# shunkenney/DPE-MVS

Hardware: AMD Instinct MI355X
Metric: depth-map Mpixels/sec (9-view 1600x1200 PatchMatch) at 1/2/4/8 GPUs; L1 vs ref (higher is better)
Workload: dtype f32; 1 GPU; DTU-like 1600x1200, 9 src views, full-res REFINE_ITER pass + geometric consistency (BASELINE configs[2]); width=1600, height=1200, num_images=10, parallelism=reference-image sharding x1

## Files before the change

dpe-mvs_amd/csrc/lds_layout.h:

```cpp
#pragma once

#if defined(__HIPCC__)
#define LDS_HD __host__ __device__
#else
#define LDS_HD
#endif

namespace dpe {
namespace lds {

constexpr int kMaxViews = 31;

struct Region {
  int off, len, align;
};

template <int N>
constexpr bool regions_ok(const Region (&r)[N], int total) {
  for (int i = 0; i < N; ++i) {
    if (r[i].len < 0 || r[i].off < 0 || r[i].off + r[i].len > total) return false;
    if (r[i].align > 1 && r[i].off % r[i].align != 0) return false;
    for (int j = i + 1; j < N; ++j)
      if (r[i].len > 0 && r[j].len > 0 && r[i].off < r[j].off + r[j].len && r[j].off < r[i].off + r[i].len) return false;
  }
// ... 4 lines not shown
struct StrongCarve {
  static constexpr int kPatch = 108;
  LDS_HD static constexpr int ib_ints(int nv) { return 2 * C + 17 + nv; }
  LDS_HD static constexpr int hyp() { return 0; }
  LDS_HD static constexpr int patch() { return P * 20; }
  LDS_HD static constexpr int cost(int) { return P * 128; }
  LDS_HD static constexpr int sp(int nv) { return P * (128 + (C + 1) * nv); }
  LDS_HD static constexpr int ref(int nv) { return P * (128 + (C + 2) * nv); }
  LDS_HD static constexpr int fc(int nv) { return P * (128 + (C + 7) * nv); }
  LDS_HD static constexpr int sums(int nv) { return P * (136 + (C + 7) * nv); }
  LDS_HD static constexpr int vw(int nv) { return P * (140 + (C + 7) * nv); }
  LDS_HD static constexpr int ib(int nv) { return P * (148 + (C + 7) * nv); }
  LDS_HD static constexpr int base(int nv) { return (ib(nv) + P * ib_ints(nv) + 3) & ~3; }
  LDS_HD static constexpr int cpl(int nv) { return base(nv); }
  LDS_HD static constexpr int alias(int nv) { return base(nv) + P * (C + 1) * 4; }
  LDS_HD static constexpr int tail(int nv) { return alias(nv) + P * (C + 1); }
  LDS_HD static constexpr int rnd(int nv) { return tail(nv) + TAIL_JOBS * 18; }
  LDS_HD static constexpr int total(int nv) { return rnd(nv) + P * 12; }
  static constexpr int IB_POS = 0;
  static constexpr int IB_FIN = C;
  static constexpr int IB_MISC = C + 8;
  static constexpr int IB_SEL = C + 16;
  LDS_HD static constexpr int ib_slots(int nv) { return C + 16 + nv; }
  static constexpr int MI_NSEL = 0, MI_JOBS = 1, MI_DEPTH = 2;

  static constexpr bool ok(int nv) {
    const Region r[] = {{hyp(), P * 20, 4},        {patch(), P * kPatch, 1}, {cost(nv), P * (C + 1) * nv, 1},
                        {sp(nv), P * nv, 1},       {ref(nv), P * 5 * nv, 1}, {fc(nv), P * 8, 1},
                        {sums(nv), P * 4, 1},      {vw(nv), P * 8, 1},       {ib(nv), P * ib_ints(nv), 1},
                        {cpl(nv), P * (C + 1) * 4, 4}, {alias(nv), P * (C + 1), 1}, {tail(nv), TAIL_JOBS * 18, 1},
                        {rnd(nv), P * 12, 1}};
    return regions_ok(r, total(nv)) && ib_slots(nv) + C + 1 == ib_ints(nv) && P * C == 64 && MI_DEPTH + 5 <= 8;
  }
  static constexpr bool ok_all() {
    for (int nv = 1; nv <= kMaxViews; ++nv) if (!ok(nv)) return false;
    return true;
  }
};

template <bool PRE>
struct WeakCarveT {
  static constexpr int PW = 0;
  static constexpr int TC = 108;
  static constexpr int TN = 180;
  static constexpr int SUMS = 324;
  static constexpr int RC = 351;
  static constexpr int OSUM = 352;
  static constexpr int CPL = 356;
  static constexpr int HYP = 388;
  static constexpr int RSUM = HYP;
  static constexpr int FC = 416;
  static constexpr int MISC = 424;
  static constexpr int NBL = 440;
  static constexpr int NBOX_A = 449;
  static constexpr int NSV = 452;
  static constexpr int NBOX_B = 461;
  static constexpr int ALIAS = PRE ? 472 : 464;
  static constexpr int VWL = PRE ? 464 : 472;
  static constexpr int RND = 472;
  static constexpr int FIXED = PRE ? 484 : 480;
  static constexpr int M_NSEL = 0, M_RADC = 1, M_INCC = 2, M_NC = 3, M_WNORM = 4, M_CMASK = 5, M_NB3 = 6, M_POOL = 7, M_FLAGS = 8;
  LDS_HD static constexpr int cost(int) { return FIXED; }
  LDS_HD static constexpr int sp(int nv) { return FIXED + 8 * nv; }
  LDS_HD static constexpr int sel(int nv) { return FIXED + 9 * nv; }
  LDS_HD static constexpr int hv(int nv) { return FIXED + 10 * nv; }
  LDS_HD static constexpr int per_pixel(int nv) { return (FIXED + 17 * nv + 3) & ~3; }

  static constexpr bool ok(int nv) {
    const Region r[] = {{PW, 108, 1},   {TC, 72, 1},      {TN, 144, 1},    {SUMS, 27, 1},       {RC, 1, 1},
                        {OSUM, 3, 1},   {CPL, 32, 4},     {HYP, 28, 4},    {FC, 8, 1},          {MISC, 16, 1},
                        {NBL, 9, 1},    {NBOX_A, 3, 1},   {NSV, 9, 1},     {NBOX_B, 1, 1},
                        {PRE ? RND : ALIAS, PRE ? 12 : 8, 1},
                        {VWL, 8, 1},    {cost(nv), 8 * nv, 1}, {sp(nv), nv, 1}, {sel(nv), nv, 1}, {hv(nv), 7 * nv, 1}};
    return regions_ok(r, per_pixel(nv)) && per_pixel(nv) % 4 == 0 && M_FLAGS + 8 <= 16 &&
           (!PRE || (ALIAS >= RND && ALIAS + 8 <= RND + 12));
  }
  static constexpr bool ok_all() {
    for (int nv = 1; nv <= kMaxViews; ++nv) if (!ok(nv)) return false;
    return true;
  }
};
using WeakCarve = WeakCarveT<false>;

static_assert(StrongCarve<4, 16, 16>::ok_all(), "strong-sweep LDS carve (edge mode): overlap, alignment or bounds");
static_assert(StrongCarve<8, 8, 16>::ok_all(), "strong-sweep LDS carve (ACMH mode): overlap, alignment or bounds");
static_assert(WeakCarveT<false>::ok_all(), "weak-sweep LDS carve: overlap, alignment or bounds");
static_assert(WeakCarveT<true>::ok_all(), "weak-sweep LDS carve (DPE_WEAK_PRE): overlap, alignment or bounds");
static_assert(4 * StrongCarve<4, 16, 16>::total(kMaxViews) * 4 <= 160 * 1024, "strong-sweep workgroup LDS (edge)");
static_assert(4 * StrongCarve<8, 8, 16>::total(kMaxViews) * 4 <= 160 * 1024, "strong-sweep workgroup LDS (ACMH)");
static_assert(4 * (4 * 4 * WeakCarveT<false>::per_pixel(9) * 4) <= 160 * 1024, "weak-sweep LDS: 4 workgroups per CU at 9 views");
static_assert(4 * (4 * 4 * WeakCarveT<true>::per_pixel(9) * 4) <= 160 * 1024, "weak-sweep LDS (DPE_WEAK_PRE): 4 workgroups per CU at 9 views");

}
}
```

dpe-mvs_amd/csrc/pass_common.h:

```cpp
#pragma once
#include "device_math.h"
#include "bres_walk.h"
#include "../../include/dpe_mvs.h"

namespace dpe {

struct ViewConst { float M[9]; float b[3]; };

struct PassConst {
  int W, H, N, LW, LH;
  int half_rows;
  uint32_t seed32, salt;
  float kinv0, kinv4, kc2, kc5;
  float gn_cos, gn_sin, gn_thr;
  int gn_shift;
  uint32_t gn_shift_m;
  int weak_nn;
  DpePatchMatchParams P;
  DpeCamera cams[DPE_MAX_IMAGES];
  ViewConst vc[DPE_MAX_IMAGES];
};

struct DevBufs {
  const float4* imgq[DPE_MAX_IMAGES];
  const uint8_t* img8; uint32_t img8_view;
// ... 200 lines not shown
}
DEV float4 random_normal_from(const DpeCamera& c, int px, int py, const float* n0, float depth) {
  float4 n = make_float4(n0[0], n0[1], n0[2], 0.0f);
  const float4 vd = view_direction(c, px, py, depth);
  if (n.x * vd.x + n.y * vd.y + n.z * vd.z > 0.0f) { n.x = -n.x; n.y = -n.y; n.z = -n.z; }
  normalize3(n);
  return n;
}
DEV float4 perturbed_normal_from(const DpeCamera& c, int px, int py, const float4& normal, const float* sc) {
  const float4 vd = view_direction(c, px, py, 1.0f);
  const float s1 = sc[0], c1 = sc[1], s2 = sc[2], c2 = sc[3], s3 = sc[4], c3 = sc[5];
  const float R0 = c2 * c3, R1 = c3 * s1 * s2 - c1 * s3, R2 = s1 * s3 + c1 * c3 * s2;
  const float R3 = c2 * s3, R4 = c1 * c3 + s1 * s2 * s3, R5 = c1 * s2 * s3 - c3 * s1;
  const float R6 = -s2, R7 = c2 * s1, R8 = c1 * c2;
  float4 np = make_float4(R0 * normal.x + R1 * normal.y + R2 * normal.z,
                          R3 * normal.x + R4 * normal.y + R5 * normal.z,
                          R6 * normal.x + R7 * normal.y + R8 * normal.z, normal.w);
  if (np.x * vd.x + np.y * vd.y + np.z * vd.z >= 0.0f) np = normal;
  normalize3(np);
  return np;
}

struct Homog { float h[9]; };
DEV Homog make_homography(const PassConst& pc, int v, const float4& pl) {
  const float iw = 1.0f / pl.w;
  const float qx = pl.x * iw, qy = pl.y * iw, qz = pl.z * iw;
  const float g0 = qx * pc.kinv0;
  const float g1 = qy * pc.kinv4;
  const float g2 = __builtin_fmaf(-qx, pc.kc2, __builtin_fmaf(-qy, pc.kc5, qz));
  const ViewConst& vc = pc.vc[v];
  Homog H;
  H.h[0] = __builtin_fmaf(-vc.b[0], g0, vc.M[0]);
  H.h[1] = __builtin_fmaf(-vc.b[0], g1, vc.M[1]);
  H.h[2] = __builtin_fmaf(-vc.b[0], g2, vc.M[2]);
  H.h[3] = __builtin_fmaf(-vc.b[1], g0, vc.M[3]);
  H.h[4] = __builtin_fmaf(-vc.b[1], g1, vc.M[4]);
  H.h[5] = __builtin_fmaf(-vc.b[1], g2, vc.M[5]);
  H.h[6] = __builtin_fmaf(-vc.b[2], g0, vc.M[6]);
  H.h[7] = __builtin_fmaf(-vc.b[2], g1, vc.M[7]);
  H.h[8] = __builtin_fmaf(-vc.b[2], g2, vc.M[8]);
  return H;
}
DEV float2 project_h(const Homog& H, float x, float y) {
  const float px = __builtin_fmaf(H.h[1], y, __builtin_fmaf(H.h[0], x, H.h[2]));
  const float py = __builtin_fmaf(H.h[4], y, __builtin_fmaf(H.h[3], x, H.h[5]));
  const float pz = __builtin_fmaf(H.h[7], y, __builtin_fmaf(H.h[6], x, H.h[8]));
  const float iz = 1.0f / pz;
  return make_float2(px * iz, py * iz);
}

DEV bool rcp_range_ok(const Homog& H, float x0, float x1, float y0, float y1) {
  const float b0 = __builtin_fmaf(H.h[6], x0, H.h[8]), b1 = __builtin_fmaf(H.h[6], x1, H.h[8]);
  const float q00 = __builtin_fmaf(H.h[7], y0, b0), q01 = __builtin_fmaf(H.h[7], y1, b0);
  const float q10 = __builtin_fmaf(H.h[7], y0, b1), q11 = __builtin_fmaf(H.h[7], y1, b1);
  const float mn = __builtin_fminf(__builtin_fminf(q00, q01), __builtin_fminf(q10, q11));
  const float mx = __builtin_fmaxf(__builtin_fmaxf(q00, q01), __builtin_fmaxf(q10, q11));
  const float amax = __builtin_fmaxf(__builtin_fmaxf(__builtin_fabsf(b0), __builtin_fabsf(b1)),
                                     __builtin_fmaxf(__builtin_fabsf(mn), __builtin_fabsf(mx)));
  const float lo = mn > 0.0f ? mn : -mx;
  return (mn > 0.0f || mx < 0.0f) && lo > amax * 9.5367431640625e-07f && lo > 7.888609052210118e-31f &&
         amax < 1.2676506002282294e+30f;
}

DEV bool taps_unclamped(const Homog& H, float x0, float x1, float y0, float y1, float wm1, float hm1) {
  const float b0 = __builtin_fmaf(H.h[6], x0, H.h[8]), b1 = __builtin_fmaf(H.h[6], x1, H.h[8]);
// ... 298 lines not shown
  if (rcp_range_ok(H, (float)(cx - radius), (float)(cx + radius), (float)(cy - radius), (float)(cy + radius)))
    generic_taps<U8, true>(pc, B, v, H, cx, cy, rcp, radius, increment, a);
  else
    generic_taps<U8, false>(pc, B, v, H, cx, cy, rcp, radius, increment, a);
  if (B.cnt) { const unsigned long long n = (unsigned long long)(2 * radius / increment + 1); count_work(B, 0, n * n); }
  return ncc_finalize(a[0], a[1], a[5], a[2], a[3], a[4]);
}

DEV float2 project_h_fast(const Homog& H, float x, float y) {
  const float px = __builtin_fmaf(H.h[1], y, __builtin_fmaf(H.h[0], x, H.h[2]));
  const float py = __builtin_fmaf(H.h[4], y, __builtin_fmaf(H.h[3], x, H.h[5]));
  const float pz = __builtin_fmaf(H.h[7], y, __builtin_fmaf(H.h[6], x, H.h[8]));
  const float iz = d_rcp_fast(pz);
  return make_float2(px * iz, py * iz);
}
template <bool FAST = false>
DEV bool center_outside(const PassConst& pc, int v, const Homog& H, int px, int py) {
  const float2 pt = FAST ? project_h_fast(H, (float)px, (float)py) : project_h(H, (float)px, (float)py);
  const DpeCamera& sc = pc.cams[v];
  return pt.x >= (float)sc.width || pt.x < 0.0f || pt.y >= (float)sc.height || pt.y < 0.0f;
}

template <int U8>
DEV float ncc_old_generic(const PassConst& pc, const DevBufs& B, int px, int py, int v, const float4& pl) {
  const Homog H = make_homography(pc, v, pl);
  count_work(B, 1, 0);
  if (center_outside(pc, v, H, px, py)) return 2.0f;
  const float rc = ref_texel(B.ref, pc.W, pc.H, px, py);
  return patch_ncc_generic<U8>(pc, B, v, H, px, py, rc, pc.P.strong_radius, pc.P.strong_increment);
}

struct Patch36 {
  float w[36], wr[36];
  float s_ref, s_rr, s_w;
  int px, py;
};
DEV void make_patch36(Patch36& P, const PassConst& pc, const DevBufs& B, int px, int py) {
  const int W = pc.W, Hh = pc.H;
  const float ss = pc.P.sigma_spatial, sc = pc.P.sigma_color;
  const float rc = ref_texel(B.ref, W, Hh, px, py);
  P.px = px; P.py = py;
  float s_ref = 0, s_rr = 0, s_w = 0;
#pragma unroll
  for (int a = 0; a < 6; ++a) {
    const int i = -5 + 2 * a;
    float r_ref = 0, r_rr = 0, r_w = 0;
#pragma unroll
    for (int b = 0; b < 6; ++b) {
      const int j = -5 + 2 * b;
      const float rp = ref_texel(B.ref, W, Hh, px + i, py + j);
      const float w = bilateral_weight(i, j, rp, rc, ss, sc);
      const float wr = w * rp;
// ... 173 lines not shown
```

dpe-mvs_amd/csrc/pass_refine.h:

```cpp
#pragma once
#include "pass_common.h"

namespace dpe {

DEV void wave_sync() {
  __builtin_amdgcn_fence(__ATOMIC_RELEASE, "wavefront");
  __builtin_amdgcn_wave_barrier();
  __builtin_amdgcn_fence(__ATOMIC_ACQUIRE, "wavefront");
}

template <int S>
DEV void patch_lds_build(float* pw, const PassConst& pc, const DevBufs& B, int px, int py, int t) {
  constexpr int R = (36 + S - 1) / S;
  const float rc = ref_texel(B.ref, pc.W, pc.H, px, py);
  float rp[R];
#pragma unroll
  for (int r = 0; r < R; ++r) {
    const int k = t + r * S < 36 ? t + r * S : 35;
    rp[r] = ref_texel(B.ref, pc.W, pc.H, px - 5 + 2 * (k / 6), py - 5 + 2 * (k % 6));
  }
#pragma unroll
  for (int r = 0; r < R; ++r) {
    const int k = t + r * S;
    if (k >= 36) break;
// ... 117 lines not shown
    r3[0] = r_sr.x; r3[1] = r_ss; r3[2] = r_sr.y;
  } else {
    const float bx = __builtin_fmaf(H.h[0], x, H.h[2]) * kTexUnit;
    const float by = __builtin_fmaf(H.h[3], x, H.h[5]) * kTexUnit;
    const float bz = __builtin_fmaf(H.h[6], x, H.h[8]);
    float r_src = 0, r_ss = 0, r_rs = 0;
#pragma unroll
    for (int b = 0; b < 6; ++b) {
      const float y = (float)(py - 5 + 2 * b);
      const float qx = __builtin_fmaf(H.h[1], y, bx);
      const float qy = __builtin_fmaf(H.h[4], y, by);
      const float iz = rcp_tap<FAST>(__builtin_fmaf(H.h[7], y, bz));
      const float sp = sample_src<U8>(B, v, W, Hh, qx, qy, iz);
      const float w = pw[2 * (a * 6 + b)], wr = pw[2 * (a * 6 + b) + 1];
      r_src = __builtin_fmaf(w, sp, r_src);
      const float ws = w * sp;
      r_ss = __builtin_fmaf(ws, sp, r_ss);
      r_rs = __builtin_fmaf(wr, sp, r_rs);
    }
    r3[0] = r_src; r3[1] = r_ss; r3[2] = r_rs;
  }
}
template <int U8>
DEV float ncc_old_lds(const float* pw, float s_ref, float s_rr, float s_w, int px, int py, const PassConst& pc,
                      const DevBufs& B, int v, const float4& pl) {
  const Homog H = make_homography(pc, v, pl);
  if (center_outside(pc, v, H, px, py)) { count_work(B, 1, 0); return 2.0f; }
  count_work(B, 1, 36);
  float a[3];
  const bool ok = rcp_range_ok(H, (float)(px - 5), (float)(px + 5), (float)(py - 5), (float)(py + 5));
  PATCH_STAT(ok);
  if (ok) {
    const bool ncl = taps_unclamped(H, (float)(px - 5), (float)(px + 5), (float)(py - 5), (float)(py + 5), (float)(pc.W - 1),
                                    (float)(pc.H - 1));
#if DPE_POOL_STATS
    atomicAdd(&g_pool[6][2], ncl ? 0ull : 1ull);
    atomicAdd(&g_pool[7][0], 1ull);
#endif
    if (DPE_UNCLAMPED && U8 != TEX_F32 && __all(ncl)) {
#if DPE_POOL_STATS
      atomicAdd(&g_pool[7][1], 1ull);
#endif
      lds_taps<U8, true, false>(pw, px, py, pc, B, v, H, a);
    } else
      lds_taps<U8, true>(pw, px, py, pc, B, v, H, a);
  } else
    lds_taps<U8, false>(pw, px, py, pc, B, v, H, a);
  return ncc_finalize_pre(s_ref, s_rr, s_w, a[0], a[1], a[2]);
}

template <int U8>
DEV float ncc_old_any(bool fast, const float* pw, float s_ref, float s_rr, float s_w, int px, int py,
                      const PassConst& pc, const DevBufs& B, int v, const float4& pl) {
  if (fast) return ncc_old_lds<U8>(pw, s_ref, s_rr, s_w, px, py, pc, B, v, pl);
  return ncc_old_generic<U8>(pc, B, px, py, v, pl);
}

DEV void baseline_and_weights(const PassConst& pc, uint32_t sel, const uint8_t* vw, float& base_line, float& weight_normal,
                              int& valid) {
  const DpeCamera& c0 = pc.cams[0];
  base_line = 0.0f; weight_normal = 0.0f; valid = 0;
  for (int si = 1; si < pc.N; ++si) {
    const int vi = si - 1;
    if (isSet(sel, vi)) {
      weight_normal += vw[vi];
      const DpeCamera& cs = pc.cams[si];
      const float d0 = c0.c[0] - cs.c[0], d1 = c0.c[1] - cs.c[1], d2 = c0.c[2] - cs.c[2];
      const float tv = d0 * d0 + d1 * d1 + d2 * d2;
      base_line += __builtin_sqrtf(tv);
      valid++;
    }
  }
}

DEV uint8_t d2w_class(const PassConst& pc, const float* pcs, uint64_t is_peak) {
  const int radius = 30;
  const int peak_count = __popcll(is_peak);
  int min_peak = 0;
// ... 319 lines not shown
```

dpe-mvs_amd/csrc/pass_sweep.h:

```cpp
#pragma once
#include "pass_common.h"
#include "pass_refine.h"
#include "lds_layout.h"

namespace dpe {

template <int MODE> constexpr int list_count() { return MODE == 0 ? 4 : 1; }
template <int MODE> DEV int list_rows(const PassConst& pc) { return MODE == 1 ? pc.H : pc.half_rows; }
template <int MODE> DEV int list_key(const PassConst& pc, const DevBufs& B, int x, int y) {
  if constexpr (MODE == 2) return (((x + y) & 1) == 0 && B.weak_rel[y * pc.W + x] == 0) ? 0 : -1;
  const bool wk = B.weak[y * pc.W + x] == DPE_WEAK;
  if constexpr (MODE == 1) return wk ? 0 : -1;
  else return (((x + y) & 1) << 1) | (wk ? 1 : 0);
}
template <int MODE>
__global__ void k_list_count(const PassConst* __restrict__ pcp, DevBufs B, int* __restrict__ row_counts) {
  constexpr int NL = list_count<MODE>();
  const PassConst& pc = *pcp;
  const int wave = threadIdx.x >> 6, lane = threadIdx.x & 63;
  const int y = blockIdx.x * 4 + wave, rows = list_rows<MODE>(pc);
  if (y >= rows) return;
  int cnt[NL];
  for (int j = 0; j < NL; ++j) cnt[j] = 0;
  for (int x0 = 0; x0 < pc.W; x0 += 64) {
// ... 298 lines not shown
      return cmp;
    }
  }
}

constexpr int kTailJobs = 16;
template <int P, int C> using StrongCarveT = lds::StrongCarve<P, C, kTailJobs>;
__host__ __device__ inline int strong_lds_per_wave(int P, int C, int nv) {
  return P == 4 && C == 16 ? StrongCarveT<4, 16>::total(nv) : StrongCarveT<8, 8>::total(nv);
}

template <int P>
DEV bool job_decode(const int* cnt, int j, int& p, int& r) {
  r = j;
#pragma unroll
  for (int q = 0; q < P; ++q) {
    if (r < cnt[q]) { p = q; return true; }
    r -= cnt[q];
  }
  return false;
}

constexpr int kBwStrong = 2;
template <int U8, bool EDGE>
__global__ void __launch_bounds__(64 * kBwStrong, kTapWaves) k_strong_coop(const PassConst* __restrict__ pcp, DevBufs B, int iter,
                                                     const int* __restrict__ list, const int* __restrict__ nlist_p) {
  extern __shared__ float4 lds4[];
  float* lds = (float*)lds4;
  const int nlist = *nlist_p;
  constexpr int C = EDGE ? 16 : 8;
  constexpr int P = 64 / C;
  const PassConst& pc = *pcp;
  const int wave = threadIdx.x >> 6, lane = threadIdx.x & 63;
  const int ps = lane / C, c = lane % C;
  const int W = pc.W, nv = pc.N - 1;
  const DpeCamera& c0 = pc.cams[0];
  const int wbase = (xcd_remap(blockIdx.x, gridDim.x, B.xcd_rows * 16) * kBwStrong + wave) * P;
  if (wbase >= nlist) return;
  const int gi = wbase + ps;
  const bool active = gi < nlist;
  const int center = active ? list[gi] : 0;
  const int x = center % W, y = center / W;
  using SC = StrongCarveT<P, C>;
  float* wl = lds + (size_t)wave * SC::total(nv);
  float4* hyp_all = (float4*)(wl + SC::hyp());
  float* pw_all = wl + SC::patch();
// ... 27 lines not shown
  bool on_edge = false;
  PHASE_BEGIN();
  if (active) {
    if (fast) patch_lds_build<C>(pw, pc, B, x, y, c);
    PHASE(14);
    int pos;
    if constexpr (EDGE) {
      on_edge = B.edge[center] != 0;
      const int d = c & 7, kind = c >> 3;
      pos = (kind == 1 && on_edge) ? -1 : edge_candidate(pc, B, costs_s, x, y, center, iter, d, kind, on_edge);
    } else {
      pos = acmh_candidate(pc, costs_s, x, y, center, c);
    }
    posl[c] = pos;
    auto phash = [](const float4& p) -> int {
      uint32_t h = __float_as_uint(p.x) * 0x9E3779B1u;
      h = (h ^ (h >> 15) ^ __float_as_uint(p.y)) * 0x85EBCA77u;
      h = (h ^ (h >> 13) ^ __float_as_uint(p.z)) * 0xC2B2AE3Du;
      h = (h ^ (h >> 16) ^ __float_as_uint(p.w)) * 0x27D4EB2Fu;
      return (int)((h ^ (h >> 15)) & 0x7FFFFFFFu);
    };
    if (pos >= 0) { const float4 pl = planes_s[pos]; cpl[c] = pl; alias[c] = phash(pl); }
    else alias[c] = (int)(0x80000000u | (uint32_t)c);
    if (c == 0) { const float4 pl = planes_s[center]; cpl[C] = pl; alias[C] = phash(pl); }
  }
  wave_sync();
  PHASE(0);
  auto same = [](const float4& a, const float4& b) {
    return __float_as_uint(a.x) == __float_as_uint(b.x) && __float_as_uint(a.y) == __float_as_uint(b.y) &&
           __float_as_uint(a.z) == __float_as_uint(b.z) && __float_as_uint(a.w) == __float_as_uint(b.w);
  };
  int al[2] = {-1, -1};
  if (active) {
#pragma unroll
    for (int r = 0; r < 2; ++r) {
      const int sl = c + r * C;
      if (sl > C || (sl < C && posl[sl] < 0)) continue;
      const float4 me = cpl[sl];
      const uint32_t h = (uint32_t)alias[sl];
      uint32_t m = 0;
#pragma unroll
      for (int t = 0; t < C; ++t) m |= ((uint32_t)alias[t] == h && t < sl) ? (1u << t) : 0u;
      int a = sl;
      while (m) {
        const int t = __builtin_ctz(m);
        if (same(cpl[t], me)) { a = t; break; }
        m &= m - 1;
      }
      al[r] = a;
    }
  }
  wave_sync();
  if (active) {
    alias[c] = al[0];
    if (c == 0) alias[C] = al[1];
  }
  wave_sync();
  PHASE(1);
  if (c == 0) {
    int n = 0;
    if (active) {
      for (int k = 0; k <= C; ++k) if (alias[k] == k) slots[n++] = k;
      if (fast) patch_lds_pre(pw, sums_all[ps * 4 + 0], sums_all[ps * 4 + 1], sums_all[ps * 4 + 2]);
    }
    misc[SC::MI_JOBS] = n;
  }
  wave_sync();
  PHASE(2);
  {
    int cnt[P], S = 0;
#pragma unroll
    for (int q = 0; q < P; ++q) { cnt[q] = ib_all[q * ibs + SC::IB_MISC + 1]; S += cnt[q]; }
    int q, r;
    const int total = S * nv, tail = total & 63;
    const bool split = fast && tail > 0 && tail <= kTailJobs;
    POOL_STAT(0, total);
    const int jend = split ? total - tail : total;
    for (int j = lane; j < jend; j += 64) {
      job_decode<P>(cnt, j % S, q, r);
      const int* iq = ib_all + q * ibs;
      const int slot = iq[SC::ib_slots(nv) + r], v = j / S + 1;
      const int cq = list[wbase + q];
      const int qx = cq % W, qy = cq / W;
      const float4 pl = cpl_all[q * (C + 1) + slot];
      const float* sm = sums_all + q * 4;
      cost_all[(q * (C + 1) + slot) * nv + v - 1] =
          ncc_old_any<U8>(fast, pw_all + q * 108, sm[0], sm[1], sm[2], qx, qy, pc, B, v, pl);
    }
    if (split) {
      float* tb = wl + SC::tail(nv);
      const int rpp = 64 / tail >= 6 ? 1 : 2, npc = 6 / rpp;
      if (lane < tail * npc) {
        const int j = jend + lane / npc, a0 = (lane % npc) * rpp;
        job_decode<P>(cnt, j % S, q, r);
        const int slot = ib_all[q * ibs + SC::ib_slots(nv) + r], v = j / S + 1;
        const int cq = list[wbase + q];
        const int qx = cq % W, qy = cq / W;
        const Homog H = make_homography(pc, v, cpl_all[q * (C + 1) + slot]);
        if (!center_outside(pc, v, H, qx, qy)) {
          const bool fr = rcp_range_ok(H, (float)(qx - 5), (float)(qx + 5), (float)(qy - 5), (float)(qy + 5));
          for (int a = a0; a < a0 + rpp; ++a) {
            float* r3 = tb + ((lane / npc) * 6 + a) * 3;
            if (fr) lds_row<U8, true>(pw_all + q * 108, qx, qy, pc, B, v, H, a, r3);
            else lds_row<U8, false>(pw_all + q * 108, qx, qy, pc, B, v, H, a, r3);
          }
        }
      }
      wave_sync();
      if (lane < tail) {
        const int j = jend + lane;
        job_decode<P>(cnt, j % S, q, r);
        const int slot = ib_all[q * ibs + SC::ib_slots(nv) + r], v = j / S + 1;
        const int cq = list[wbase + q];
        const Homog H = make_homography(pc, v, cpl_all[q * (C + 1) + slot]);
        float cst = 2.0f;
        if (center_outside(pc, v, H, cq % W, cq / W)) {
          count_work(B, 1, 0);
        } else {
          count_work(B, 1, 36);
          float s_src = 0, s_ss = 0, s_rs = 0;
          for (int a = 0; a < 6; ++a) {
            const float* r3 = tb + (lane * 6 + a) * 3;
            s_src += r3[0]; s_ss += r3[1]; s_rs += r3[2];
          }
          const float* sm = sums_all + q * 4;
          cst = ncc_finalize_pre(sm[0], sm[1], sm[2], s_src, s_ss, s_rs);
        }
        cost_all[(q * (C + 1) + slot) * nv + v - 1] = cst;
      }
    }
  }
  wave_sync();
  PHASE(3);
  if (active) {
    for (int sl = c; sl <= C; sl += C) {
      const int a = alias[sl];
      if (a >= 0 && a != sl)
        for (int v = 0; v < nv; ++v) cost[sl * nv + v] = cost[a * nv + v];
    }
// ... 99 lines not shown
      const float db = depth_from_plane(c0, cand, x, y);
      if (db >= pc.P.depth_min && db <= pc.P.depth_max && fc[mi] < cost_now) {
        depth_now = db; pnow = cand; cost_now = fc[mi]; B.sel[center] = tsv;
      }
    }
  }
  wave_sync();
  if (active && c == 0) {
    const float dmin = pc.P.depth_min, dmax = pc.P.depth_max;
    const float depth_rand = rnd[0] * (dmax - dmin) + dmin;
    const float4 prand = random_normal_from(c0, x, y, rnd + 1, depth_now);
    const float dminp = (1 - 0.02f) * depth_now, dmaxp = (1 + 0.02f) * depth_now;
    const float depth_perturbed = rnd[4] * (dmaxp - dminp) + dminp;
    const float4 ppert = perturbed_normal_from(c0, x, y, pnow, rnd + 5);
    float4 h0 = pnow, h1 = prand, h2 = prand, h3 = ppert, h4 = pnow;
    h0.w = dist2origin(c0, x, y, depth_rand, h0);
    h1.w = dist2origin(c0, x, y, depth_now, h1);
    h2.w = dist2origin(c0, x, y, depth_rand, h2);
    h3.w = dist2origin(c0, x, y, depth_now, h3);
    h4.w = dist2origin(c0, x, y, depth_perturbed, h4);
    hyp[0] = h0; hyp[1] = h1; hyp[2] = h2; hyp[3] = h3; hyp[4] = h4;
  }
  wave_sync();
  PHASE(9);
  {
    int cnt[P];
#pragma unroll
    for (int q = 0; q < P; ++q) cnt[q] = 5 * ib_all[q * ibs + SC::IB_MISC];
    POOL_STAT(1, [&] { int t = 0; for (int q = 0; q < P; ++q) t += cnt[q]; return t; }());
    int q, r;
    for (int j = lane; job_decode<P>(cnt, j, q, r); j += 64) {
      const int* iq = ib_all + q * ibs;
      const int h = r % 5, k = r / 5;
      const int cq = list[wbase + q];
      const float* sm = sums_all + q * 4;
      ref_all[(q * 5 + h) * nv + k] = ncc_old_any<U8>(fast, pw_all + q * 108, sm[0], sm[1], sm[2], cq % W, cq / W, pc,
                                                      B, iq[SC::IB_SEL + k] + 1, hyp_all[q * 5 + h]);
    }
  }
  wave_sync();
  PHASE(10);
  if (active && c < 5) {
    const int h = c;
    float tc = 0.0f;
    for (int k = 0; k < nsel; ++k) tc += vwl[sel_list[k]] * ref[h * nv + k];
    tc /= sums_all[ps * 4 + 3];
    fc[h] = tc;
    misc[SC::MI_DEPTH + h] = __float_as_int(depth_from_plane(c0, hyp[h], x, y));
  }
  wave_sync();
  PHASE(13);
  if (active && c == 0) {
    const float dmin = pc.P.depth_min, dmax = pc.P.depth_max;
    for (int h = 0; h < 5; ++h) {
      const float tc = fc[h], db = __int_as_float(misc[SC::MI_DEPTH + h]);
      if (db >= dmin && db <= dmax && tc < cost_now) { depth_now = db; pnow = hyp[h]; cost_now = tc; }
    }
    if (pc.P.state == DPE_REFINE_INIT) {
      if ((double)cost_now < (double)cost_written - 0.1) { B.costs[center] = cost_now; B.planes[center] = pnow; }
    } else {
// ... 153 lines not shown
    if (!nfast && !T.tab_n) WSTAT(16);
    if (nfast) {
      float a[3];
      tab_taps<U8, true, 3>(pc, B, v, H, np.x, np.y, T.rad_n, T.inc_n, 3, T.tn + (k - 1) * 18, a);
      count_work(B, 0, 9ull);
      const float* sm = T.sums + 3 * k;
      tc = ncc_finalize_pre(sm[0], sm[1], sm[2], a[0], a[1], a[2]);
    } else {
      tc = T.tab_n ? patch_ncc_tab<U8, 6>(pc, B, v, H, np.x, np.y, T.rad_n, T.inc_n, T.n_n, T.tn + (k - 1) * 18,
                                       T.sums + 3 * k)
                   : patch_ncc_generic<U8>(pc, B, v, H, np.x, np.y, T.rc, T.rad_n, T.inc_n);
    }
    strong_cost += tc; strong_count++;
  }
  if (strong_count == 0) return center_cost;
  strong_cost /= (float)strong_count;
  strong_cost = MINo(strong_cost, 2.0f);
  return (float)(0.25 * (double)center_cost + 0.75 * (double)strong_cost);
}

using WC = lds::WeakCarveT<true>;
constexpr int kWeakFixed = WC::FIXED;
__host__ __device__ inline int weak_lds_per_pixel(int nv) { return WC::per_pixel(nv); }

template <int U8, int C>
__global__ void __launch_bounds__(256, kTapWaves) k_weak_coop(const PassConst* __restrict__ pcp, DevBufs B, int iter,
                                                   const int* __restrict__ list, const int* __restrict__ nlist_p) {
  extern __shared__ float4 lds4[];
  static_assert(C == 16 || C == 32, "the per-pixel phases give lanes 0..8 the patch sums and lanes 8..15 the alias rows");
  constexpr int P = 64 / C;
  const PassConst& pc = *pcp;
  const int nlist = *nlist_p;
  const int wpb = blockDim.x >> 6;
  const int wave = threadIdx.x >> 6, lane = threadIdx.x & 63;
  const int ps = lane / C, c = lane % C;
  const int W = pc.W, Hh = pc.H, nv = pc.N - 1;
  const DpeCamera& c0 = pc.cams[0];
  const int wgbase = xcd_remap(blockIdx.x, gridDim.x, B.xcd_rows * 16) * wpb * P;
  const int wbase = wgbase + wave * P;
  constexpr bool WGP = true;
  if ((WGP ? wgbase : wbase) >= nlist) return;
  const int gi = wbase + ps;
  const bool active = gi < nlist;
  const int center = active ? list[gi] : 0;
  const int x = center % W, y = center / W;
  const int S = weak_lds_per_pixel(nv);
// ... 147 lines not shown
    }
  }
  wave_sync();
  PHASE(0);
  T.nb3 = false;
  if (active && T.tab_n && T.n_n == 3) {
    int x0 = 0x7FFFFFFF, x1 = -0x7FFFFFFF, y0 = 0x7FFFFFFF, y1 = -0x7FFFFFFF;
    for (int k = 1; k < DPE_NEIGHBOUR_NUM; ++k) {
      const short2 np = nbl[k];
      if (np.x == -1 || np.y == -1) continue;
      x0 = min(x0, (int)np.x); x1 = max(x1, (int)np.x); y0 = min(y0, (int)np.y); y1 = max(y1, (int)np.y);
    }
    if (x0 <= x1) {
      T.nb3 = true;
      T.nbox[0] = (float)(x0 - T.rad_n); T.nbox[1] = (float)(x1 + T.rad_n);
      T.nbox[2] = (float)(y0 - T.rad_n); T.nbox[3] = (float)(y1 + T.rad_n);
    }
  }
  if (active) {
    if (c == C - 2) {
      misc[WC::M_RADC] = T.rad_c; misc[WC::M_INCC] = T.inc_c; misc[WC::M_NC] = T.n_c; misc[WC::M_NB3] = T.nb3 ? 1 : 0;
      pb[WC::NBOX_A] = T.nbox[0]; pb[WC::NBOX_A + 1] = T.nbox[1]; pb[WC::NBOX_A + 2] = T.nbox[2]; pb[WC::NBOX_B] = T.nbox[3];
      pb[WC::RC] = T.rc;
    }
    if (rows1 && c == 0) {
      const short2 np = nbl[0];
      if (!(np.x == -1 || np.y == -1)) {
        float a_ref = 0, a_rr = 0, a_w = 0;
        for (int a = 0; a < n_c; ++a) {
          const float* rs3 = pb + WC::RSUM + 3 * a;
          a_ref += rs3[0]; a_rr += rs3[1]; a_w += rs3[2];
        }
        ncc_pre(a_ref, a_rr, a_w, sums[0], sums[1], sums[2]);
      }
    }
    for (int k = c; k < 9; k += C) {
      const short2 np = nbl[k];
      if (rows1 || np.x == -1 || np.y == -1 || !(k == 0 ? tab_c : tab_n)) continue;
      const int n = k == 0 ? n_c : n_n, rad = k == 0 ? rad_c : rad_n, inc = k == 0 ? inc_c : inc_n;
      const float* tp = k == 0 ? tcp : tnp + (k - 1) * 18;
      float a_ref = 0, a_rr = 0, a_w = 0;
      for (int a = 0; a < n; ++a) {
        float r_ref = 0, r_rr = 0, r_w = 0;
        for (int b = 0; b < n; ++b) {
          const float rp = ref_texel(B.ref, W, Hh, np.x - rad + a * inc, np.y - rad + b * inc);
          const float w = tp[2 * (a * n + b)], wr = tp[2 * (a * n + b) + 1];
// ... 12 lines not shown
        const float4 me = cpl[i];
        for (int t = 0; t < i; ++t)
          if (misc[WC::M_FLAGS + t] && __float_as_uint(cpl[t].x) == __float_as_uint(me.x) &&
              __float_as_uint(cpl[t].y) == __float_as_uint(me.y) && __float_as_uint(cpl[t].z) == __float_as_uint(me.z) &&
              __float_as_uint(cpl[t].w) == __float_as_uint(me.w)) { a = t; break; }
      }
      alias[i] = a;
    }
  }
  wave_sync();
  PHASE(1);
  if (active && c == 0) {
    uint32_t um = 0;
    for (int i = 0; i < 8; ++i) if (misc[WC::M_FLAGS + i] && alias[i] == i) um |= 1u << i;
    misc[WC::M_CMASK] = (int)um;
    misc[WC::M_POOL] = __builtin_popcount(um);
  }
  if (!active && c == 0) misc[WC::M_POOL] = 0;
  pool_sync();
  {
    const int Sj = pool_total();
    int q, r;
    pool_stat_g(2, Sj * nv);
    for (int j = pl_lane; j < Sj * nv; j += pl_n) {
      pool_decode(j % Sj, q, r);
      const int v = j / Sj + 1;
      float* qb = pix(q);
      uint32_t m = (uint32_t)((const int*)(qb + WC::MISC))[WC::M_CMASK];
      for (; r > 0; --r) m &= m - 1;
      const int i = __builtin_ctz(m);
      const int cq = list[pbase + q];
      (qb + WC::cost(nv))[i * nv + v - 1] = ncc_new_tab<U8>(pc, B, tab_of(q), cq % W, cq / W, v, ((const float4*)(qb + WC::CPL))[i]);
    }
  }
  pool_sync();
  PHASE(2);
  if (active)
    for (int i = c; i < 8; i += C)
      if (misc[WC::M_FLAGS + i] && alias[i] != i)
        for (int v = 0; v < nv; ++v) cost[i * nv + v] = cost[alias[i] * nv + v];
  wave_sync();
  PHASE(3);
  const float cost_threshold = (float)(0.8 * (double)d_expf((float)(iter * iter) / (-90.0f)));
  if (active) {
    auto cst = [&](int j, int i) -> float { return cost[j * nv + i]; };
    for (int v = c; v < nv; v += C) {
      float prior = 0.0f;
      for (int i = 0; i < 8; ++i) {
        const short2 np = nbl[i + 1];
        if (np.x == -1 || np.y == -1) continue;
        prior += isSet(nsv[i + 1], v) == 1 ? 0.9f : 0.1f;
      }
      sp[v] = view_prob_raw(cst, v, cost_threshold) * prior;
    }
  }
// ... 2 lines not shown
  Rng rs;
  rng_init(rs, (uint32_t)center, pc.seed32, STREAM_ITER_BASE + 4 * iter + 2, pc.salt);
  view_sample_coop(sp, (int*)hv, nv, c, C, active, rs, vwl, B.vw + (size_t)center * DPE_MAX_IMAGES);
  uint32_t tsv = 0; float wnorm = 0.0f;
  if (active && c == 0) {
    rng_seek(rs, 15);
    int ns = 0;
    for (int i = 0; i < nv; ++i) if (vwl[i] > 0) { setBit(tsv, i); wnorm += vwl[i]; sel_list[ns++] = i; }
    misc[WC::M_NSEL] = ns;
    misc[WC::M_WNORM] = __float_as_int(wnorm);
    const float4 f6 = B.fit_plane[center];
    hyp[6] = f6;
    misc[WC::M_POOL] = ((f6.x == 0 && f6.y == 0 && f6.z == 0) ? 1 : 2) * ns;
  }
  if (!active && c == 0) misc[WC::M_POOL] = 0;
  pool_sync();
  PHASE(5);
  const int nsel = active ? misc[WC::M_NSEL] : 0;
  const float wn = active ? __int_as_float(misc[WC::M_WNORM]) : 1.0f;
  const float4 cur = active ? B.planes[center] : make_float4(0, 0, 0, 1);
  const float4 fp = active ? B.fit_plane[center] : make_float4(0, 0, 0, 0);
  const bool has_fit = !(fp.x == 0 && fp.y == 0 && fp.z == 0);
  auto hyp_val_q = [&](int q, int v, const float4& pl) __attribute__((always_inline)) -> float {
    const int cq = list[pbase + q];
    const int qx = cq % W, qy = cq / W;
    const float cn = ncc_new_tab<U8>(pc, B, tab_of(q), qx, qy, v, pl);
    return geom ? cn + gf * geom_cost(pc, B, qx, qy, v, pl) : cn;
  };
  {
    const int tot = pool_total();
    pool_stat_g(3, tot);
    int q, r;
    for (int j = pl_lane; j < tot; j += pl_n) {
      pool_decode(j, q, r);
      float* qb = pix(q);
      const int ns = ((const int*)(qb + WC::MISC))[WC::M_NSEL];
      const int h = r / ns, k = r % ns;
      const int v = ((const int*)(qb + WC::sel(nv)))[k] + 1;
      (qb + WC::hv(nv))[h * nv + k] = hyp_val_q(q, v, h ? ((const float4*)(qb + WC::HYP))[6] : B.planes[list[pbase + q]]);
    }
  }
  PHASE(12);
  if (active) {
    for (int i = c; i < 8; i += C) {
      const bool fl = misc[WC::M_FLAGS + i] != 0;
      const float3 fwi = (geom && fl) ? geom_point(pc, x, y, cpl[i]) : make_float3(0.0f, 0.0f, 0.0f);
      float f = 0.0f;
      for (int j = 0; j < nv; ++j) {
        const int w = vwl[j];
        if (w > 0) {
          if (geom) {
            if (fl) f += w * (cost[i * nv + j] + gf * geom_cost_at(pc, B, x, y, j + 1, fwi));
            else f += w * (cost[i * nv + j] + gf * 3.0f);
          } else {
            f += w * cost[i * nv + j];
          }
        }
      }
      fc[i] = f / wn;
    }
// ... 38 lines not shown
    const float4 prand = random_normal_from(c0, x, y, rnd + 1, depth_now);
    const float dminp = (1 - 0.02f) * depth_now, dmaxp = (1 + 0.02f) * depth_now;
    const float depth_perturbed = rnd[4] * (dmaxp - dminp) + dminp;
    const float4 ppert = perturbed_normal_from(c0, x, y, pnow, rnd + 5);
    float4 h0 = pnow, h1 = prand, h2 = prand, h3 = ppert, h4 = pnow;
    h0.w = dist2origin(c0, x, y, depth_rand, h0);
    h1.w = dist2origin(c0, x, y, depth_now, h1);
    h2.w = dist2origin(c0, x, y, depth_rand, h2);
    h3.w = dist2origin(c0, x, y, depth_now, h3);
    h4.w = dist2origin(c0, x, y, depth_perturbed, h4);
    hyp[0] = h0; hyp[1] = h1; hyp[2] = h2; hyp[3] = h3; hyp[4] = h4;
  }
  if (c == 0) misc[WC::M_POOL] = active && has_fit ? 5 * nsel : 0;
  pool_sync();
  PHASE(7);
  {
    const int tot = pool_total();
    pool_stat_g(4, tot);
    int q, r;
    for (int j = pl_lane; j < tot; j += pl_n) {
      pool_decode(j, q, r);
      float* qb = pix(q);
      const int ns = ((const int*)(qb + WC::MISC))[WC::M_NSEL];
      const int h = r / ns, k = r % ns;
      const int v = ((const int*)(qb + WC::sel(nv)))[k] + 1;
      (qb + WC::hv(nv))[(2 + h) * nv + k] = hyp_val_q(q, v, ((const float4*)(qb + WC::HYP))[h]);
    }
  }
  pool_sync();
  PHASE(8);
  if (active && c == 0) {
    if (has_fit) {
      for (int h = 0; h < 5; ++h) {
        const float4 tp = hyp[h];
        float tc = 0.0f;
        for (int k = 0; k < nsel; ++k) tc += vwl[sel_list[k]] * hv[(2 + h) * nv + k];
        tc /= wnorm;
        const float db = depth_from_plane(c0, tp, x, y);
        if (db >= dmin && db <= dmax && tc < cost_now) { depth_now = db; pnow = tp; cost_now = tc; }
      }
    }
    float4 fin = cur;
    if (pc.P.state == DPE_REFINE_INIT) {
      if ((double)cost_now < (double)cost_written - 0.1) { fin = pnow; B.planes[center] = pnow; }
    } else {
      fin = pnow;
      B.planes[center] = pnow;
    }
    hyp[5] = fin;
  }
  if (c == 0) misc[WC::M_POOL] = active ? nsel : 0;
  pool_sync();
  PHASE(9);
  {
    const int tot = pool_total();
    pool_stat_g(5, tot);
    int q, r;
    for (int j = pl_lane; j < tot; j += pl_n) {
      pool_decode(j, q, r);
      float* qb = pix(q);
      const int cq = list[pbase + q];
      const int v = ((const int*)(qb + WC::sel(nv)))[r] + 1;
      (qb + WC::hv(nv))[r] = ncc_old_any<U8>(fast_old, qb + WC::PW, qb[WC::OSUM], qb[WC::OSUM + 1], qb[WC::OSUM + 2], cq % W,
                                                   cq / W, pc, B, v, ((const float4*)(qb + WC::HYP))[5]);
    }
  }
  pool_sync();
  PHASE(10);
  if (active && c == 0) {
    float c2 = 0.0f;
    for (int k = 0; k < nsel; ++k) c2 += vwl[sel_list[k]] * hv[k];
    B.costs[center] = c2 / wnorm;
  }
  PHASE(11);
  PHASE_END(1);
}

}
```

Measured before the change: 30.71 Mpix/s.

## Hoist per-plane homography terms and cache pixel coords in LDS for sweep jobs

The plane-dependent homography terms (reciprocal of w, the g0/g1/g2 products) are now computed once per unique plane and stored in LDS, so each per-view job only does the nine view-dependent FMAs. Packed pixel x|y coordinates are cached in LDS so jobs no longer reload the list and do integer div/mod by W. Job index decoding uses incremental remainder and quotient counters instead of per-iteration division, and the h/k split uses conditional subtraction. This trades a few extra LDS slots and a sync against repeated divides and global loads. A static assert also pins strong-sweep residency at 9 views.

```diff
diff --git a/dpe-mvs_amd/csrc/lds_layout.h b/dpe-mvs_amd/csrc/lds_layout.h
--- a/dpe-mvs_amd/csrc/lds_layout.h
+++ b/dpe-mvs_amd/csrc/lds_layout.h
@@ -50,7 +50,8 @@
   static constexpr int IB_MISC = C + 8;
   static constexpr int IB_SEL = C + 16;
   LDS_HD static constexpr int ib_slots(int nv) { return C + 16 + nv; }
-  static constexpr int MI_NSEL = 0, MI_JOBS = 1, MI_DEPTH = 2;
+  static constexpr int MI_NSEL = 0, MI_JOBS = 1, MI_DEPTH = 2, MI_XY = 7;
+  LDS_HD static constexpr int hg(int nv) { return cpl(nv); }
 
   static constexpr bool ok(int nv) {
     const Region r[] = {{hyp(), P * 20, 4},        {patch(), P * kPatch, 1}, {cost(nv), P * (C + 1) * nv, 1},
@@ -58,7 +59,8 @@
                         {sums(nv), P * 4, 1},      {vw(nv), P * 8, 1},       {ib(nv), P * ib_ints(nv), 1},
                         {cpl(nv), P * (C + 1) * 4, 4}, {alias(nv), P * (C + 1), 1}, {tail(nv), TAIL_JOBS * 18, 1},
                         {rnd(nv), P * 12, 1}};
-    return regions_ok(r, total(nv)) && ib_slots(nv) + C + 1 == ib_ints(nv) && P * C == 64 && MI_DEPTH + 5 <= 8;
+    return regions_ok(r, total(nv)) && ib_slots(nv) + C + 1 == ib_ints(nv) && P * C == 64 && MI_DEPTH + 5 <= MI_XY &&
+           MI_XY < 8 && 5 <= C + 1 ;
   }
   static constexpr bool ok_all() {
     for (int nv = 1; nv <= kMaxViews; ++nv) if (!ok(nv)) return false;
@@ -83,6 +85,7 @@
   static constexpr int NBOX_A = 449;
   static constexpr int NSV = 452;
   static constexpr int NBOX_B = 461;
+  static constexpr int XY = 462;
   static constexpr int ALIAS = PRE ? 472 : 464;
   static constexpr int VWL = PRE ? 464 : 472;
   static constexpr int RND = 472;
@@ -97,7 +100,7 @@
   static constexpr bool ok(int nv) {
     const Region r[] = {{PW, 108, 1},   {TC, 72, 1},      {TN, 144, 1},    {SUMS, 27, 1},       {RC, 1, 1},
                         {OSUM, 3, 1},   {CPL, 32, 4},     {HYP, 28, 4},    {FC, 8, 1},          {MISC, 16, 1},
-                        {NBL, 9, 1},    {NBOX_A, 3, 1},   {NSV, 9, 1},     {NBOX_B, 1, 1},
+                        {NBL, 9, 1},    {NBOX_A, 3, 1},   {NSV, 9, 1},     {NBOX_B, 1, 1},  {XY, 1, 1},
                         {PRE ? RND : ALIAS, PRE ? 12 : 8, 1},
                         {VWL, 8, 1},    {cost(nv), 8 * nv, 1}, {sp(nv), nv, 1}, {sel(nv), nv, 1}, {hv(nv), 7 * nv, 1}};
     return regions_ok(r, per_pixel(nv)) && per_pixel(nv) % 4 == 0 && M_FLAGS + 8 <= 16 &&
@@ -116,6 +119,9 @@
 static_assert(WeakCarveT<true>::ok_all(), "weak-sweep LDS carve (DPE_WEAK_PRE): overlap, alignment or bounds");
 static_assert(4 * StrongCarve<4, 16, 16>::total(kMaxViews) * 4 <= 160 * 1024, "strong-sweep workgroup LDS (edge)");
 static_assert(4 * StrongCarve<8, 8, 16>::total(kMaxViews) * 4 <= 160 * 1024, "strong-sweep workgroup LDS (ACMH)");
+constexpr int kStrongWgWaves = 2;
+static_assert(8 * (kStrongWgWaves * StrongCarve<4, 16, 16>::total(9) * 4 + 1280) <= 160 * 1024,
+              "strong-sweep LDS (edge): 8 workgroups per CU at 9 views");
 static_assert(4 * (4 * 4 * WeakCarveT<false>::per_pixel(9) * 4) <= 160 * 1024, "weak-sweep LDS: 4 workgroups per CU at 9 views");
 static_assert(4 * (4 * 4 * WeakCarveT<true>::per_pixel(9) * 4) <= 160 * 1024, "weak-sweep LDS (DPE_WEAK_PRE): 4 workgroups per CU at 9 views");
 
diff --git a/dpe-mvs_amd/csrc/pass_common.h b/dpe-mvs_amd/csrc/pass_common.h
--- a/dpe-mvs_amd/csrc/pass_common.h
+++ b/dpe-mvs_amd/csrc/pass_common.h
@@ -1,6 +1,7 @@
 #pragma once
 #include "device_math.h"
 #include "bres_walk.h"
+#include "plane_terms.h"
 #include "../../include/dpe_mvs.h"
 
 namespace dpe {
@@ -247,25 +248,20 @@
 }
 
 struct Homog { float h[9]; };
-DEV Homog make_homography(const PassConst& pc, int v, const float4& pl) {
-  const float iw = 1.0f / pl.w;
-  const float qx = pl.x * iw, qy = pl.y * iw, qz = pl.z * iw;
-  const float g0 = qx * pc.kinv0;
-  const float g1 = qy * pc.kinv4;
-  const float g2 = __builtin_fmaf(-qx, pc.kc2, __builtin_fmaf(-qy, pc.kc5, qz));
+DEV PlaneG plane_terms(const PassConst& pc, const float4& pl) {
+  return plane_terms_raw(pc.kinv0, pc.kinv4, pc.kc2, pc.kc5, pl.x, pl.y, pl.z, pl.w);
+}
+DEV Homog homography_from(const PassConst& pc, int v, const PlaneG& g) {
   const ViewConst& vc = pc.vc[v];
   Homog H;
-  H.h[0] = __builtin_fmaf(-vc.b[0], g0, vc.M[0]);
-  H.h[1] = __builtin_fmaf(-vc.b[0], g1, vc.M[1]);
-  H.h[2] = __builtin_fmaf(-vc.b[0], g2, vc.M[2]);
-  H.h[3] = __builtin_fmaf(-vc.b[1], g0, vc.M[3]);
-  H.h[4] = __builtin_fmaf(-vc.b[1], g1, vc.M[4]);
-  H.h[5] = __builtin_fmaf(-vc.b[1], g2, vc.M[5]);
-  H.h[6] = __builtin_fmaf(-vc.b[2], g0, vc.M[6]);
-  H.h[7] = __builtin_fmaf(-vc.b[2], g1, vc.M[7]);
-  H.h[8] = __builtin_fmaf(-vc.b[2], g2, vc.M[8]);
+  homography_rows(vc.M, vc.b, g, H.h);
   return H;
 }
+DEV Homog make_homography(const PassConst& pc, int v, const float4& pl) {
+  return homography_from(pc, v, plane_terms(pc, pl));
+}
+DEV float4 plane_g4(const PlaneG& g) { return make_float4(g.g0, g.g1, g.g2, 0.0f); }
+DEV PlaneG plane_g_of(const float4& f) { PlaneG g; g.g0 = f.x; g.g1 = f.y; g.g2 = f.z; return g; }
 DEV float2 project_h(const Homog& H, float x, float y) {
   const float px = __builtin_fmaf(H.h[1], y, __builtin_fmaf(H.h[0], x, H.h[2]));
   const float py = __builtin_fmaf(H.h[4], y, __builtin_fmaf(H.h[3], x, H.h[5]));
@@ -610,12 +606,15 @@
 }
 
 template <int U8>
-DEV float ncc_old_generic(const PassConst& pc, const DevBufs& B, int px, int py, int v, const float4& pl) {
-  const Homog H = make_homography(pc, v, pl);
+DEV float ncc_old_generic_h(const PassConst& pc, const DevBufs& B, int px, int py, int v, const Homog& H) {
   count_work(B, 1, 0);
   if (center_outside(pc, v, H, px, py)) return 2.0f;
   const float rc = ref_texel(B.ref, pc.W, pc.H, px, py);
   return patch_ncc_generic<U8>(pc, B, v, H, px, py, rc, pc.P.strong_radius, pc.P.strong_increment);
+}
+template <int U8>
+DEV float ncc_old_generic(const PassConst& pc, const DevBufs& B, int px, int py, int v, const float4& pl) {
+  return ncc_old_generic_h<U8>(pc, B, px, py, v, make_homography(pc, v, pl));
 }
 
 struct Patch36 {
diff --git a/dpe-mvs_amd/csrc/pass_refine.h b/dpe-mvs_amd/csrc/pass_refine.h
--- a/dpe-mvs_amd/csrc/pass_refine.h
+++ b/dpe-mvs_amd/csrc/pass_refine.h
@@ -163,9 +163,8 @@
   }
 }
 template <int U8>
-DEV float ncc_old_lds(const float* pw, float s_ref, float s_rr, float s_w, int px, int py, const PassConst& pc,
-                      const DevBufs& B, int v, const float4& pl) {
-  const Homog H = make_homography(pc, v, pl);
+DEV float ncc_old_lds_h(const float* pw, float s_ref, float s_rr, float s_w, int px, int py, const PassConst& pc,
+                        const DevBufs& B, int v, const Homog& H) {
   if (center_outside(pc, v, H, px, py)) { count_work(B, 1, 0); return 2.0f; }
   count_work(B, 1, 36);
   float a[3];
@@ -191,10 +190,23 @@
 }
 
 template <int U8>
+DEV float ncc_old_lds(const float* pw, float s_ref, float s_rr, float s_w, int px, int py, const PassConst& pc,
+                      const DevBufs& B, int v, const float4& pl) {
+  return ncc_old_lds_h<U8>(pw, s_ref, s_rr, s_w, px, py, pc, B, v, make_homography(pc, v, pl));
+}
+
+template <int U8>
 DEV float ncc_old_any(bool fast, const float* pw, float s_ref, float s_rr, float s_w, int px, int py,
                       const PassConst& pc, const DevBufs& B, int v, const float4& pl) {
   if (fast) return ncc_old_lds<U8>(pw, s_ref, s_rr, s_w, px, py, pc, B, v, pl);
   return ncc_old_generic<U8>(pc, B, px, py, v, pl);
+}
+template <int U8>
+DEV float ncc_old_any_g(bool fast, const float* pw, float s_ref, float s_rr, float s_w, int px, int py,
+                        const PassConst& pc, const DevBufs& B, int v, const PlaneG& g) {
+  const Homog H = homography_from(pc, v, g);
+  if (fast) return ncc_old_lds_h<U8>(pw, s_ref, s_rr, s_w, px, py, pc, B, v, H);
+  return ncc_old_generic_h<U8>(pc, B, px, py, v, H);
 }
 
 DEV void baseline_and_weights(const PassConst& pc, uint32_t sel, const uint8_t* vw, float& base_line, float& weight_normal,
diff --git a/dpe-mvs_amd/csrc/pass_sweep.h b/dpe-mvs_amd/csrc/pass_sweep.h
--- a/dpe-mvs_amd/csrc/pass_sweep.h
+++ b/dpe-mvs_amd/csrc/pass_sweep.h
@@ -344,6 +344,7 @@
 }
 
 constexpr int kBwStrong = 2;
+static_assert(kBwStrong == lds::kStrongWgWaves, "lds_layout.h checks the 9-view residency for this workgroup size");
 template <int U8, bool EDGE>
 __global__ void __launch_bounds__(64 * kBwStrong, kTapWaves) k_strong_coop(const PassConst* __restrict__ pcp, DevBufs B, int iter,
                                                      const int* __restrict__ list, const int* __restrict__ nlist_p) {
@@ -417,7 +418,10 @@
     };
     if (pos >= 0) { const float4 pl = planes_s[pos]; cpl[c] = pl; alias[c] = phash(pl); }
     else alias[c] = (int)(0x80000000u | (uint32_t)c);
-    if (c == 0) { const float4 pl = planes_s[center]; cpl[C] = pl; alias[C] = phash(pl); }
+    if (c == 0) {
+      const float4 pl = planes_s[center]; cpl[C] = pl; alias[C] = phash(pl);
+      misc[SC::MI_XY] = x | y << 16;
+    }
   }
   wave_sync();
   PHASE(0);
@@ -452,6 +456,10 @@
   }
   wave_sync();
   PHASE(1);
+  if (active) {
+    for (int sl = c; sl <= C; sl += C)
+      if (alias[sl] == sl) cpl[sl] = plane_g4(plane_terms(pc, cpl[sl]));
+  }
   if (c == 0) {
     int n = 0;
     if (active) {
@@ -471,16 +479,21 @@
     const bool split = fast && tail > 0 && tail <= kTailJobs;
     POOL_STAT(0, total);
     const int jend = split ? total - tail : total;
+    const int Sd = S > 0 ? S : 1;
+    const int dq = 64 / Sd, dr = 64 % Sd;
+    int jr = lane % Sd, jv = lane / Sd + 1;
     for (int j = lane; j < jend; j += 64) {
-      job_decode<P>(cnt, j % S, q, r);
+      job_decode<P>(cnt, jr, q, r);
       const int* iq = ib_all + q * ibs;
-      const int slot = iq[SC::ib_slots(nv) + r], v = j / S + 1;
-      const int cq = list[wbase + q];
-      const int qx = cq % W, qy = cq / W;
-      const float4 pl = cpl_all[q * (C + 1) + slot];
+      const int slot = iq[SC::ib_slots(nv) + r], v = jv;
+      const int xy = iq[SC::IB_MISC + SC::MI_XY];
+      const int qx = xy & 0xFFFF, qy = xy >> 16;
+      const PlaneG g = plane_g_of(cpl_all[q * (C + 1) + slot]);
       const float* sm = sums_all + q * 4;
       cost_all[(q * (C + 1) + slot) * nv + v - 1] =
-          ncc_old_any<U8>(fast, pw_all + q * 108, sm[0], sm[1], sm[2], qx, qy, pc, B, v, pl);
+          ncc_old_any_g<U8>(fast, pw_all + q * 108, sm[0], sm[1], sm[2], qx, qy, pc, B, v, g);
+      jr += dr; jv += dq;
+      if (jr >= S) { jr -= S; ++jv; }
     }
     if (split) {
       float* tb = wl + SC::tail(nv);
@@ -489,9 +502,9 @@
         const int j = jend + lane / npc, a0 = (lane % npc) * rpp;
         job_decode<P>(cnt, j % S, q, r);
         const int slot = ib_all[q * ibs + SC::ib_slots(nv) + r], v = j / S + 1;
-        const int cq = list[wbase + q];
-        const int qx = cq % W, qy = cq / W;
-        const Homog H = make_homography(pc, v, cpl_all[q * (C + 1) + slot]);
+        const int xy = ib_all[q * ibs + SC::IB_MISC + SC::MI_XY];
+        const int qx = xy & 0xFFFF, qy = xy >> 16;
+        const Homog H = homography_from(pc, v, plane_g_of(cpl_all[q * (C + 1) + slot]));
         if (!center_outside(pc, v, H, qx, qy)) {
           const bool fr = rcp_range_ok(H, (float)(qx - 5), (float)(qx + 5), (float)(qy - 5), (float)(qy + 5));
           for (int a = a0; a < a0 + rpp; ++a) {
@@ -506,10 +519,10 @@
         const int j = jend + lane;
         job_decode<P>(cnt, j % S, q, r);
         const int slot = ib_all[q * ibs + SC::ib_slots(nv) + r], v = j / S + 1;
-        const int cq = list[wbase + q];
-        const Homog H = make_homography(pc, v, cpl_all[q * (C + 1) + slot]);
+        const int xy = ib_all[q * ibs + SC::IB_MISC + SC::MI_XY];
+        const Homog H = homography_from(pc, v, plane_g_of(cpl_all[q * (C + 1) + slot]));
         float cst = 2.0f;
-        if (center_outside(pc, v, H, cq % W, cq / W)) {
+        if (center_outside(pc, v, H, xy & 0xFFFF, xy >> 16)) {
           count_work(B, 1, 0);
         } else {
           count_work(B, 1, 36);
@@ -655,6 +668,9 @@
     hyp[0] = h0; hyp[1] = h1; hyp[2] = h2; hyp[3] = h3; hyp[4] = h4;
   }
   wave_sync();
+  float4* hg_all = (float4*)(wl + SC::hg(nv));
+  if (active && c < 5) hg_all[ps * 5 + c] = plane_g4(plane_terms(pc, hyp[c]));
+  wave_sync();
   PHASE(9);
   {
     int cnt[P];
@@ -665,10 +681,10 @@
     for (int j = lane; job_decode<P>(cnt, j, q, r); j += 64) {
       const int* iq = ib_all + q * ibs;
       const int h = r % 5, k = r / 5;
-      const int cq = list[wbase + q];
+      const int xy = iq[SC::IB_MISC + SC::MI_XY];
       const float* sm = sums_all + q * 4;
-      ref_all[(q * 5 + h) * nv + k] = ncc_old_any<U8>(fast, pw_all + q * 108, sm[0], sm[1], sm[2], cq % W, cq / W, pc,
-                                                      B, iq[SC::IB_SEL + k] + 1, hyp_all[q * 5 + h]);
+      ref_all[(q * 5 + h) * nv + k] = ncc_old_any_g<U8>(fast, pw_all + q * 108, sm[0], sm[1], sm[2], xy & 0xFFFF, xy >> 16,
+                                                        pc, B, iq[SC::IB_SEL + k] + 1, plane_g_of(hg_all[q * 5 + h]));
     }
   }
   wave_sync();
@@ -868,6 +884,14 @@
 using WC = lds::WeakCarveT<true>;
 constexpr int kWeakFixed = WC::FIXED;
 __host__ __device__ inline int weak_lds_per_pixel(int nv) { return WC::per_pixel(nv); }
+
+template <int NH>
+DEV void split_hk(int r, int ns, int& h, int& k) {
+  h = 0; k = r;
+#pragma unroll
+  for (int t = 1; t < NH; ++t)
+    if (k >= ns) { k -= ns; ++h; }
+}
 
 template <int U8, int C>
 __global__ void __launch_bounds__(256, kTapWaves) k_weak_coop(const PassConst* __restrict__ pcp, DevBufs B, int iter,
@@ -1061,6 +1085,7 @@
       misc[WC::M_RADC] = T.rad_c; misc[WC::M_INCC] = T.inc_c; misc[WC::M_NC] = T.n_c; misc[WC::M_NB3] = T.nb3 ? 1 : 0;
       pb[WC::NBOX_A] = T.nbox[0]; pb[WC::NBOX_A + 1] = T.nbox[1]; pb[WC::NBOX_A + 2] = T.nbox[2]; pb[WC::NBOX_B] = T.nbox[3];
       pb[WC::RC] = T.rc;
+      ((int*)pb)[WC::XY] = x | y << 16;
     }
     if (rows1 && c == 0) {
       const short2 np = nbl[0];
@@ -1119,15 +1144,20 @@
     const int Sj = pool_total();
     int q, r;
     pool_stat_g(2, Sj * nv);
+    const int Sd = Sj > 0 ? Sj : 1;
+    const int dq = pl_n / Sd, dr = pl_n % Sd;
+    int jr = pl_lane % Sd, jv = pl_lane / Sd + 1;
     for (int j = pl_lane; j < Sj * nv; j += pl_n) {
-      pool_decode(j % Sj, q, r);
-      const int v = j / Sj + 1;
+      pool_decode(jr, q, r);
+      const int v = jv;
       float* qb = pix(q);
       uint32_t m = (uint32_t)((const int*)(qb + WC::MISC))[WC::M_CMASK];
       for (; r > 0; --r) m &= m - 1;
       const int i = __builtin_ctz(m);
-      const int cq = list[pbase + q];
-      (qb + WC::cost(nv))[i * nv + v - 1] = ncc_new_tab<U8>(pc, B, tab_of(q), cq % W, cq / W, v, ((const float4*)(qb + WC::CPL))[i]);
+      const int xy = ((const int*)qb)[WC::XY];
+      (qb + WC::cost(nv))[i * nv + v - 1] = ncc_new_tab<U8>(pc, B, tab_of(q), xy & 0xFFFF, xy >> 16, v, ((const float4*)(qb + WC::CPL))[i]);
+      jr += dr; jv += dq;
+      if (jr >= Sj) { jr -= Sj; ++jv; }
     }
   }
   pool_sync();
@@ -1176,8 +1206,8 @@
   const float4 fp = active ? B.fit_plane[center] : make_float4(0, 0, 0, 0);
   const bool has_fit = !(fp.x == 0 && fp.y == 0 && fp.z == 0);
   auto hyp_val_q = [&](int q, int v, const float4& pl) __attribute__((always_inline)) -> float {
-    const int cq = list[pbase + q];
-    const int qx = cq % W, qy = cq / W;
+    const int xy = ((const int*)pix(q))[WC::XY];
+    const int qx = xy & 0xFFFF, qy = xy >> 16;
     const float cn = ncc_new_tab<U8>(pc, B, tab_of(q), qx, qy, v, pl);
     return geom ? cn + gf * geom_cost(pc, B, qx, qy, v, pl) : cn;
   };
@@ -1189,7 +1219,8 @@
       pool_decode(j, q, r);
       float* qb = pix(q);
       const int ns = ((const int*)(qb + WC::MISC))[WC::M_NSEL];
-      const int h = r / ns, k = r % ns;
+      int h, k;
+      split_hk<2>(r, ns, h, k);
       const int v = ((const int*)(qb + WC::sel(nv)))[k] + 1;
       (qb + WC::hv(nv))[h * nv + k] = hyp_val_q(q, v, h ? ((const float4*)(qb + WC::HYP))[6] : B.planes[list[pbase + q]]);
     }
@@ -1274,7 +1305,8 @@
       pool_decode(j, q, r);
       float* qb = pix(q);
       const int ns = ((const int*)(qb + WC::MISC))[WC::M_NSEL];
-      const int h = r / ns, k = r % ns;
+      int h, k;
+      split_hk<5>(r, ns, h, k);
       const int v = ((const int*)(qb + WC::sel(nv)))[k] + 1;
       (qb + WC::hv(nv))[(2 + h) * nv + k] = hyp_val_q(q, v, ((const float4*)(qb + WC::HYP))[h]);
     }
@@ -1311,10 +1343,10 @@
     for (int j = pl_lane; j < tot; j += pl_n) {
       pool_decode(j, q, r);
       float* qb = pix(q);
-      const int cq = list[pbase + q];
+      const int xy = ((const int*)qb)[WC::XY];
       const int v = ((const int*)(qb + WC::sel(nv)))[r] + 1;
-      (qb + WC::hv(nv))[r] = ncc_old_any<U8>(fast_old, qb + WC::PW, qb[WC::OSUM], qb[WC::OSUM + 1], qb[WC::OSUM + 2], cq % W,
-                                                   cq / W, pc, B, v, ((const float4*)(qb + WC::HYP))[5]);
+      (qb + WC::hv(nv))[r] = ncc_old_any<U8>(fast_old, qb + WC::PW, qb[WC::OSUM], qb[WC::OSUM + 1], qb[WC::OSUM + 2], xy & 0xFFFF,
+                                                   xy >> 16, pc, B, v, ((const float4*)(qb + WC::HYP))[5]);
     }
   }
   pool_sync();
diff --git a/dpe-mvs_amd/csrc/plane_terms.h b/dpe-mvs_amd/csrc/plane_terms.h
--- /dev/null
+++ b/dpe-mvs_amd/csrc/plane_terms.h
@@ -0,0 +1,35 @@
+#pragma once
+
+#if defined(__HIPCC__)
+#define PT_HD __host__ __device__
+#else
+#define PT_HD
+#endif
+
+namespace dpe {
+
+struct PlaneG { float g0, g1, g2; };
+
+PT_HD inline PlaneG plane_terms_raw(float kinv0, float kinv4, float kc2, float kc5, float nx, float ny, float nz, float w) {
+  const float iw = 1.0f / w;
+  const float qx = nx * iw, qy = ny * iw, qz = nz * iw;
+  PlaneG g;
+  g.g0 = qx * kinv0;
+  g.g1 = qy * kinv4;
+  g.g2 = __builtin_fmaf(-qx, kc2, __builtin_fmaf(-qy, kc5, qz));
+  return g;
+}
+
+PT_HD inline void homography_rows(const float* M, const float* b, const PlaneG& g, float* h) {
+  h[0] = __builtin_fmaf(-b[0], g.g0, M[0]);
+  h[1] = __builtin_fmaf(-b[0], g.g1, M[1]);
+  h[2] = __builtin_fmaf(-b[0], g.g2, M[2]);
+  h[3] = __builtin_fmaf(-b[1], g.g0, M[3]);
+  h[4] = __builtin_fmaf(-b[1], g.g1, M[4]);
+  h[5] = __builtin_fmaf(-b[1], g.g2, M[5]);
+  h[6] = __builtin_fmaf(-b[2], g.g0, M[6]);
+  h[7] = __builtin_fmaf(-b[2], g.g1, M[7]);
+  h[8] = __builtin_fmaf(-b[2], g.g2, M[8]);
+}
+
+}
```

New measurement: 30.66 Mpix/s. About the same (-0.2%).
